# l13039968960/stm32H7-YOLO

Measured on AMD Instinct MI355X. Metric: images/sec int8 YOLO-face 56x56, higher is better.
Workload: dtype int8; 1 GPU; BASELINE configs[1]: batch=4096 int8 YOLO-face 56x56x3 frames per GPU, fused LDS-resident forward + GPU box decode; frames_per_gpu=4096, global_batch=4096, frame_bytes_in=9408, frame_bytes_out=882, input_batches_rotated=8, input_bytes_resident=308281344, kernel=yoloface56_fused<F=2,NW=8>, requant_rounding=ref, parallelism=single GPU, gather_every=1, collectives_issued=0, launch_streams=2

## Files before the change

stm32h7-yolo_amd/csrc/yf_fused56.hip.h:

```cpp


template <class B, int C, int F, int NT>
__device__ __forceinline__ void dump_buf(const char* frames, int8_t* dump, long stride, long off, long first_frame,
                                         long n_frames, int tid, int ch0 = 0, int split = 1 << 30, int gap = 0) {
  if (!dump) return;
  for (int i = tid; i < F * B::P * C; i += NT) {
    const int ch = i % C; const int t = i / C;
    const int p = t % B::P; const int f = t / B::P;
    if (first_frame + f >= n_frames) continue;
    const int phys = ch0 + ch + (ch >= split ? gap : 0);
    dump[(first_frame + f) * stride + off + (long)p * C + ch] = (int8_t)frames[f * B::FS + B::at_p(p) + phys];
  }
}

template <class B, int C, int FT, int NT, class IdOf>
__device__ __forceinline__ void dump_sets(const char* frames, int8_t* dump, long stride, long off, const IdOf& id_of, int tid, int ch0 = 0, int split = 1 << 30, int gap = 0) {
  for (int i = tid; i < FT * B::P * C; i += NT) {
    const int ch = i % C; const int t = i / C;
    const int p = t % B::P; const int f = t / B::P;
    const long id = id_of(f);
    if (id < 0) continue;
    const int phys = ch0 + ch + (ch >= split ? gap : 0);
    dump[id * stride + off + (long)p * C + ch] = (int8_t)frames[f * B::FS + B::at_p(p) + phys];
  }
}

struct DumpOffsets {
  enum { T1 = 0, T2 = T1 + 6272, T3 = T2 + 6272, T4 = T3 + 3136, Q21 = T4 + 14112, T6 = Q21 + 3528, T7 = T6 + 3528,
         T8 = T7 + 1176, T9 = T8 + 7056, T11 = T9 + 7056, T14 = T11 + 1176, T15 = T14 + 7056, Q45 = T15 + 4704,
         T17 = Q45 + 1176, T18 = T17 + 1176, T19 = T18 + 392, T20 = T19 + 1960, T22 = T20 + 1960, T23 = T22 + 392,
         T24 = T23 + 1960, T26 = T24 + 1960, T30 = T26 + 392, T31 = T30 + 2352, T32 = T31 + 1960, T33 = T32 + 1960,
         P8 = T33 + 1568, C17 = P8 + 3528, P25 = C17 + 1176, C34 = P25 + 1176, C40 = C34 + 392, L43 = C40 + 392,
         TOTAL = L43 + 1176 };
};

struct NetParams {
  const int8_t* in;
  int8_t* out;
  long n;
  const uint8_t* tab;
  int8_t* dump;
  int stop_stage;
  yf_det* dets;
  int* counts;
  int cap, mode;
  int q_thr;
  float w_scale, h_scale;
  char* scratch;
};
static_assert(sizeof(yf_table_index) <= YF_INDEX_RESERVED, "index does not fit its reserved slot");
typedef const __attribute__((address_space(4))) char* kargs_ptr;
__device__ __forceinline__ kargs_ptr kargs_here() {
  kargs_ptr p = (kargs_ptr)__builtin_amdgcn_kernarg_segment_ptr();
  asm volatile("" : "+s"(p));
  return p;
}
#define YF_ARG(FIELD) (*reinterpret_cast<const __attribute__((address_space(4))) decltype(NetParams::FIELD)*>(kargs_here() + offsetof(NetParams, FIELD)))

#ifndef YF_POOL_MERGE
#define YF_POOL_MERGE 1
#endif
#ifndef YF_POOL8H_WAVES
#define YF_POOL8H_WAVES 3
#endif
#ifndef YF_POOL8V_WAVES
#define YF_POOL8V_WAVES 3
#endif
#ifndef YF_PRIO_LIST
#define YF_PRIO_LIST 3,3,3,3,3,3,3,3,3,3, 2,2,2,2, 1,1,1,1,1,1, 0,0,0,0,0,0,0
#endif
constexpr int STAGE_PRIO[27] = {YF_PRIO_LIST};
template <int K> __device__ __forceinline__ void stage_prio() {
  if constexpr (K == 0 || STAGE_PRIO[K] != STAGE_PRIO[K - 1]) __builtin_amdgcn_s_setprio(STAGE_PRIO[K]);
}
#if defined(YF_LAB) && defined(YF_DUMP_PROD_ORDER)
#define YF_PDUMP 1
#else
#define YF_PDUMP 0
#endif
template <bool DUMP> constexpr bool tail_batch() { return !DUMP || YF_PDUMP; }

template <int F, int NW, bool DUMP, bool CAM = false>
#if !defined(YF_LAB) || !defined(YF_TPJ13)
#undef YF_TPJ13
#define YF_TPJ13 3
#endif
#if !defined(YF_LAB) || !defined(YF_TPJ23)
#undef YF_TPJ23
#define YF_TPJ23 2
#endif
#if defined(YF_LAB) && defined(YF_WHATIF_WPE)
#define YF_WPE(NW) YF_WHATIF_WPE
#else
#define YF_WPE(NW) ((NW) == 12 ? 6 : (NW) >= 8 ? 4 : ((NW) == 6 ? 3 : 2))
#endif
__global__ void __launch_bounds__(NW * 64, YF_WPE(NW)) yoloface56_fused(const NetParams prm) {
  extern __shared__ __attribute__((aligned(16))) char smem[];
  constexpr int NT = NW * 64;
  constexpr bool BATCH = tail_batch<DUMP>();
  constexpr bool POOL_MERGE = YF_POOL_MERGE != 0 && (!DUMP || YF_PDUMP) && NW >= 8;
  constexpr bool XDUMP = DUMP && !YF_PDUMP;
  typedef Buf<B_T14::OFF, 14, 14, 32, 14, 0, 0> B_T6X;
  typedef typename std::conditional<POOL_MERGE, B_T6X, B_T6>::type B_T6M;
  constexpr int FT = BATCH ? 2 * F : F;
  typedef TailBufs<BATCH ? FRAME_STRIDE / 2 : FRAME_STRIDE> U;
  constexpr int OUT_ALL_BYTES = BATCH ? 0 : (F * OUT_FRAME_BYTES + 15) & ~15;
  static_assert(std::is_same<decltype(&yoloface56_fused<F, NW, DUMP, CAM>), void (*)(const NetParams)>::value, "YF_ARG: NetParams is the kernel's only argument (kernarg offset 0)");
  uint8_t* luts = reinterpret_cast<uint8_t*>(smem);
  constexpr int PRE = v2::pre_bytes<F, tail_batch<DUMP>()>();
  char* out_all = smem + PRE;
  char* frames = smem + PRE + OUT_ALL_BYTES;
  const int n_frames = (int)prm.n;
  const int tid0 = threadIdx.x;
  const uint8_t* __restrict__ tab = prm.tab;
  int vz = 0;
  asm volatile("" : "+v"(vz));
  const __attribute__((address_space(1))) uint8_t* lut_src = (const __attribute__((address_space(1))) uint8_t*)(tab + PLAN.lut_off);
  asm volatile("" : "+s"(lut_src));
  for (int i = tid0; i < v2::LUT_B / 16; i += NT)
    reinterpret_cast<v4u*>(luts)[i] = *(const __attribute__((address_space(1))) v4u*)(lut_src + (uint32_t)(16 * i));
  for (int i = tid0; i < v2::ZERO_B / 16; i += NT) reinterpret_cast<uint4*>(smem + v2::ZERO)[i] = uint4{0, 0, 0, 0};
  constexpr int DBG_LUT = PRE + OUT_ALL_BYTES + FRAME_BYTES + (F - 1) * FRAME_STRIDE;
  if constexpr (DUMP) { if (tid0 < YF_DBG_LUT_BYTES / 16) reinterpret_cast<v4u*>(smem + DBG_LUT)[tid0] = *(const __attribute__((address_space(1))) v4u*)(lut_src + (uint32_t)(YF_N_LUT * 256 + YF_ADDLUT_BYTES + 16 * tid0)); }
#if !(defined(YF_LAB) && defined(YF_WHATIF_NO_PROLOGUE_TABLES))
  {
    typedef v2::JobTabs<F, tail_batch<DUMP>()> JTS;
    typedef typename JTS::U UT;
    v2::fill_jobtab<F, 1, B_T1, B_T2, JTS::JT_DW3>(smem, tid0);
    v2::fill_jobtab<F, 2, B_T4, B_T6M, JTS::JT_DW10>(smem, tid0);
    v2::fill_jobtab<F, 1, B_T8, B_T9, JTS::JT_DW15>(smem, tid0);
    v2::fill_jobtab<JTS::FT, 2, typename UT::T15, typename UT::T17, JTS::JT_DW27>(smem, tid0);
    v2::fill_jobtab<JTS::FT, 1, typename UT::T19, typename UT::T20, JTS::JT_DW32>(smem, tid0);
    typedef v2::HaloTabs<F, tail_batch<DUMP>()> HTS;
    v2::build_halotab<typename HTS::G1, HTS::H_T1, NT>(smem, tid0);
    v2::build_halotab<typename HTS::G4, HTS::H_T4, NT>(smem, tid0);
    v2::build_halotab<typename HTS::G8, HTS::H_T8, NT>(smem, tid0);
    v2::build_halotab<typename HTS::G15, HTS::H_T15, NT>(smem, tid0);
    v2::build_halotab<typename HTS::G19, HTS::H_T19, NT>(smem, tid0);
  }
#endif

  auto sfresh = [](int v) { asm volatile("" : "+s"(v)); return v; };
  auto n_groups = [&]() { return (int)((uint32_t)(sfresh(n_frames) + F - 1) / (uint32_t)F); };
  int gstep = (int)gridDim.x;
  asm volatile("" : "+s"(gstep));
  auto park_slot = [&]() { return YF_ARG(scratch) + (uint32_t)(sfresh((int)blockIdx.x) * (F * TailBufs<FRAME_BYTES>::T15_BYTES)); };
  const AddK no_add = {};
  auto addctx = [&](int k) {
    const uint8_t* a = tab + offsetof(yf_table_index, add) + k * sizeof(yf_add);
    return AddK{uniform_u32(a + offsetof(yf_add, mo2)), uniform_u32(a + offsetof(yf_add, zro)),
                (unsigned long)uniform_u32(a + offsetof(yf_add, c64o)) | ((unsigned long)uniform_u32(a + offsetof(yf_add, c64o) + 4) << 32),
                (int)uniform_u32(a + offsetof(yf_add, rso))};
  };
  constexpr long DS = DumpOffsets::TOTAL;
#ifdef YF_BARPROF
  bool prof_on = false;
  int bar_no = 0;
  long long* prof_out = reinterpret_cast<long long*>(prm.dump) + ((long)blockIdx.x * NW + __builtin_amdgcn_readfirstlane(tid0 >> 6)) * 80;
#define YF_SYNC() do { asm volatile("s_waitcnt vmcnt(0)" ::: "memory");    \
                       if (prof_on && (tid0 & 63) == 0 && bar_no < 40) prof_out[2 * bar_no] = __builtin_readcyclecounter(); __syncthreads(); \
                       if (prof_on && (tid0 & 63) == 0 && bar_no < 40) prof_out[2 * bar_no + 1] = __builtin_readcyclecounter(); ++bar_no; } while (0)
#else
#define YF_SYNC() do { asm volatile("s_waitcnt vmcnt(0)" ::: "memory"); __syncthreads(); } while (0)
#endif
#define YF_HALO(B, RING, FR, G, HOFF, WI, TID) \
  do { int ht_ = TID; asm volatile("" : "+v"(ht_)); \
       v2::fill_halo_t<B, typename v2::HaloTabs<F, BATCH>::G, v2::HaloTabs<F, BATCH>::HOFF>(frames, load_halo_zp(tab, WI), ht_); } while (0)
#define YF_FETCH(CS, WV, LN) v2::fetch_consts_s<CS>(tab, WV, LN)
#define YF_CONV1(WV, LN, CS) v2::conv1_2_stage<F, NW, CS>(frames, tab, WV, LN)
#define YF_DENSE(FR, TPJ, KS, BW, IN, OUT, CH0, COUT, EPI, LUT, ADDB, DI, AD, WV, LN, CS) \
  v2::dense2_stage<FR, NW, TPJ, KS, BW, IN, OUT, CH0, COUT, EPI, LUT, ADDB, CS>(frames, out_all, tab, AD, WV, LN)
#define YF_DW(FR, STRIDE, IN, OUT, C, LUT, WI, WV, LN, CS, JTOFF) v2::dw2_stage<FR, NW, STRIDE, IN, OUT, C, LUT, CS, v2::JobTabs<F, BATCH>::JTOFF>(frames, tab, WV, LN)
#define YF_DUMP(BUF, C, OFF, ...) \
  if constexpr (DUMP) { if (prm.dump) { dump_buf<BUF, C, F, NT>(frames, prm.dump, DS, DumpOffsets::OFF, first, n_frames, tid, ##__VA_ARGS__); YF_SYNC(); } }
  int stage_no = 0;
#define YF_STAGE_END() if constexpr (DUMP) { if (++stage_no == prm.stop_stage) continue; }
#define YF_PRIO(K) stage_prio<K>()

  int prev_first = -1;
  auto decode_prev = [&](int w, int ln) {
    if (prm.dets != nullptr && prev_first >= 0 && w >= NW - F && prev_first + (w - (NW - F)) < n_frames) {
      int dl = ln;
      asm volatile("" : "+v"(dl));
      yfdec::decode_frame(reinterpret_cast<const int8_t*>(out_all) + (w - (NW - F)) * OUT_FRAME_BYTES, prev_first + (w - (NW - F)), dl,
                          prm.mode, prm.w_scale, prm.h_scale, prm.dets, prm.counts, prm.cap);
    }
  };
  constexpr int PARKED = (int)0x80000000;
  for (int st = blockIdx.x; (st & ~PARKED) < n_groups(); st += gstep) {
    const int grp = st & ~PARKED;
    const int first = grp * F;
#ifdef YF_BARPROF
    bar_no = 0;
    prof_on = !DUMP && prm.dump != nullptr && grp == (int)blockIdx.x + gstep;
#endif
    int tid = tid0, tid_f = tid0, tid_m = tid0, tid_t = tid0;
    if constexpr ((YF_LAUNDER & 1) != 0) asm volatile("" : "+v"(tid_f));
    if constexpr ((YF_LAUNDER & 2) != 0) asm volatile("" : "+v"(tid_m));
    if constexpr ((YF_LAUNDER & 4) != 0) asm volatile("" : "+v"(tid_t));
    const int lane = tid & 63;
    const int wave = __builtin_amdgcn_readfirstlane(tid >> 6);
    const int L_f = tid_f & 63, L_m = tid_m & 63, L_t = tid_t & 63;
    const int W_f = __builtin_amdgcn_readfirstlane(tid_f >> 6), W_m = __builtin_amdgcn_readfirstlane(tid_m >> 6), W_t = __builtin_amdgcn_readfirstlane(tid_t >> 6);
    (void)lane; (void)wave;
#if !defined(YF_BARPROF)
    asm volatile("s_waitcnt lgkmcnt(0)\n\ts_barrier" ::: "memory");
#else
    YF_SYNC();
#endif
    stage_no = 0;
    YF_PRIO(0);
    int tid_s = tid0;
    asm volatile("" : "+v"(tid_s));
    if constexpr (CAM) stage_input_cam<F, NT>(frames, reinterpret_cast<const uint8_t*>(YF_ARG(in)), first, n_frames, (int)uniform_u32(tab + offsetof(yf_table_index, in_zp)), tid_s);
    else stage_input<F, NT>(frames, YF_ARG(in), first, n_frames, (int)uniform_u32(tab + offsetof(yf_table_index, in_zp)), tid_s);
    YF_FETCH(0, W_f, L_f);
    YF_HALO(B_T1, true, F, G1, H_T1, YF_W_DW3, tid_f);
    YF_SYNC();
    YF_STAGE_END()
    YF_PRIO(1);
    YF_FETCH(1, W_f, L_f);
    YF_CONV1(W_f, L_f, 0);
    YF_SYNC(); YF_DUMP(B_T1, 8, T1)
    YF_STAGE_END()
    YF_PRIO(2);
    YF_FETCH(2, W_f, L_f);
    YF_DW(F, 1, B_T1, B_T2, 8, YF_L_LEAKY4, YF_W_DW3, W_f, L_f, 1, JT_DW3);
    YF_SYNC(); YF_DUMP(B_T2, 8, T2)
    YF_STAGE_END()
    YF_PRIO(3);
    YF_FETCH(3, W_f, L_f);
    YF_DENSE(F, 1, 1, 8, B_T2, B_T3, 0, 4, EPI_RAW, 0, B_T3, YF_D_C5, no_add, W_f, L_f, 2);
    YF_SYNC(); YF_DUMP(B_T3, 4, T3)
    YF_STAGE_END()
    YF_PRIO(4);
    YF_HALO(B_T4, false, F, G4, H_T4, YF_W_DW10, tid_f);
    YF_FETCH(4, W_f, L_f);
    YF_DENSE(F, 5, 1, 4, B_T3, B_T4, 0, 18, EPI_LUT, YF_L_LEAKY7, B_T4, YF_D_C6, no_add, W_f, L_f, 3);
    YF_SYNC(); YF_DUMP(B_T4, 18, T4)
    YF_STAGE_END()
    if constexpr (POOL_MERGE) {
      constexpr int PH = YF_POOL8H_WAVES, PV = YF_POOL8V_WAVES;
      YF_PRIO(5);
      YF_FETCH(5, W_m, L_m);
      if (W_m < PH) {
        if constexpr (F == 2) pool8_h_rows<F, PH>(frames, W_m, L_m);
        else pool8_h<F, PH * 64>(frames, tid_m);
      } else v2::dw2_stage<F, NW - PH, 2, B_T4, B_T6M, 18, YF_L_LEAKY11, 4, v2::JobTabs<F, BATCH>::JT_DW10>(frames, tab, W_m - PH, L_m);
      YF_SYNC(); YF_DUMP(B_T6M, 18, T6)
      YF_PRIO(8);
      YF_FETCH(6, W_m, L_m);
      YF_DENSE(F, 1, 2, 16, B_T6M, B_T7, 0, 6, EPI_RAW, 0, B_T7, YF_D_C12, no_add, W_m, L_m, 5);
      YF_SYNC(); YF_DUMP(B_T7, 6, T7)
      YF_PRIO(9);
      YF_HALO(B_T8, true, F, G8, H_T8, YF_W_DW15, tid_m);
      YF_FETCH(7, W_m, L_m);
      if (W_m < PV) pool8_v<F, PV * 64, false>(frames, tid_m);
      else v2::dense2_stage<F, NW - PV, YF_TPJ13, 1, 8, B_T7, B_T8, 0, 36, EPI_LUT, YF_L_LEAKY14, B_T8, 6>(frames, out_all, tab, no_add, W_m - PV, L_m);
      YF_SYNC(); YF_DUMP(B_T14, 18, Q21) YF_DUMP(B_T8, 36, T8)
    } else {
  YF_PRIO(5);
#if !(defined(YF_LAB) && defined(YF_WHATIF_NO_POOL8H))
      pool8_h<F, NT>(frames, tid_f);
      YF_SYNC();
#endif
      YF_STAGE_END()
      YF_PRIO(6);
      pool8_v<F, NT, XDUMP>(frames, tid_m);
      YF_SYNC();
      YF_PRIO(7);
      YF_FETCH(5, W_m, L_m);
      YF_DW(F, 2, B_T4, B_T6, 18, YF_L_LEAKY11, YF_W_DW10, W_m, L_m, 4, JT_DW10);
      YF_SYNC(); YF_DUMP(B_T14, 18, Q21) YF_DUMP(B_T14, 18, P8, YF_T14_CONV_BASE) YF_DUMP(B_T6, 18, T6)
      YF_STAGE_END()
      YF_PRIO(8);
      YF_FETCH(6, W_m, L_m);
      YF_DENSE(F, 1, 2, 16, B_T6, B_T7, 0, 6, EPI_RAW, 0, B_T7, YF_D_C12, no_add, W_m, L_m, 5);
      YF_SYNC(); YF_DUMP(B_T7, 6, T7)
      YF_STAGE_END()
      YF_PRIO(9);
      YF_HALO(B_T8, true, F, G8, H_T8, YF_W_DW15, tid_m);
      YF_FETCH(7, W_m, L_m);
      YF_DENSE(F, YF_TPJ13, 1, 8, B_T7, B_T8, 0, 36, EPI_LUT, YF_L_LEAKY14, B_T8, YF_D_C13, no_add, W_m, L_m, 6);
      YF_SYNC(); YF_DUMP(B_T8, 36, T8)
      YF_STAGE_END()
    }
    YF_PRIO(10);
    YF_FETCH(8, W_m, L_m);
    YF_DW(F, 1, B_T8, B_T9, 36, YF_L_LEAKY16, YF_W_DW15, W_m, L_m, 7, JT_DW15);
    YF_SYNC(); YF_DUMP(B_T9, 36, T9)
    YF_STAGE_END()
    YF_PRIO(11);
    YF_FETCH(9, W_m, L_m);
    if constexpr (XDUMP)
      v2::dense2_stage<F, NW, 1, 3, 16, B_T9, B_T11, 0, 6, EPI_ADD, YF_A_ADD18, B_T7, 8, B_T14::OFF + YF_T14_CONV_BASE, B_T14::S>(frames, out_all, tab, addctx(YF_A_ADD18), W_m, L_m);
    else
    YF_DENSE(F, 1, 3, 16, B_T9, B_T11, 0, 6, EPI_ADD, YF_A_ADD18, B_T7, YF_D_C17, addctx(YF_A_ADD18), W_m, L_m, 8);
    YF_SYNC(); YF_DUMP(B_T11, 6, T11) if constexpr (XDUMP) { YF_DUMP(B_T14, 6, C17, YF_T14_CONV_BASE) }
    YF_STAGE_END()
    YF_PRIO(12);
    YF_FETCH(10, W_m, L_m);
    YF_DENSE(F, 3, 1, 8, B_T11, B_T14, YF_T14_CONV_BASE, 18, EPI_LUT, YF_L_LEAKY20, B_T14, YF_D_C19, no_add, W_m, L_m, 9);
    YF_SYNC(); YF_DUMP(B_T14, 36, T14, 0, 18, 2)
    YF_STAGE_END()
    YF_PRIO(13);
    if constexpr (BATCH) {
#if !(defined(YF_LAB) && defined(YF_WHATIF_FS))
      static_assert(U::T15::FS >= U::T15_BYTES && B_T9::OFF <= U::T15::FS && U::T15::FS + U::T15_BYTES <= B_T14::OFF,
                    "the odd sets' T15 lands on T9 / T11 (dead), clear of conv2d_23's input (concat_22) and output (the even sets' T15)");
#endif
      if (st < 0) {
        constexpr int PV = TailBufs<FRAME_BYTES>::T15_BYTES / 16, WI = (PV + 63) / 64;
        const char* park = park_slot();
        for (int j = W_m; j < F * WI; j += NW) {
          const int f = j / WI, k0 = (j - f * WI) * 64;
          if (k0 + L_m < PV)
            __builtin_amdgcn_global_load_lds((const __attribute__((address_space(1))) void*)(uintptr_t)(park + (uint32_t)((f * PV + k0 + L_m) * 16)),
                                             (__attribute__((address_space(3))) void*)(uintptr_t)(uint32_t)(PRE + (2 * f + 1) * U::T15::FS + 16 * k0),
                                             16, 0, 0);
        }
      }
    }
    YF_HALO(B_T15, false, F, G15, H_T15, YF_W_DW27, tid_m);
    YF_FETCH(11, W_m, L_m);
    YF_DENSE(F, YF_TPJ23, 3, 16, B_T14, B_T15, 0, 24, EPI_LUT, YF_L_LEAKY24, B_T15, YF_D_C23, no_add, W_m, L_m, 10);
    if constexpr (BATCH) asm volatile("s_waitcnt vmcnt(0)" ::: "memory");
    YF_SYNC(); YF_DUMP(B_T15, 24, T15)
    YF_STAGE_END()
    int odd_first = -1;
    if constexpr (BATCH) {
      constexpr int V = U::T15_BYTES / 16;
      static_assert(U::T15_BYTES == TailBufs<FRAME_BYTES>::T15_BYTES, "one slot size for the park stores and the DMA back");
      if (st >= 0 && grp + gstep < n_groups()) {
        char* park = park_slot();
        __builtin_assume(tid_t >= 0 && tid_t < NT);
        for (int i = tid_t; i < F * V; i += NT) {
          const int f = i / V, k = i - f * V;
          *reinterpret_cast<uint4*>(park + (uint32_t)(16 * i)) = *reinterpret_cast<const uint4*>(frames + f * FRAME_STRIDE + 16 * k);
        }
        st |= PARKED;
        continue;
      }
      if (st < 0) {
        odd_first = (grp - gstep) * F;
        st &= ~PARKED;
      }
    }
    const int first_t = sfresh(grp) * F;
    auto frame_of = [&](int f) -> int {
      int id = first_t + f;
      if constexpr (BATCH) id = (f & 1) ? (odd_first >= 0 ? odd_first + (f >> 1) : -1) : first_t + (f >> 1);
      return id < n_frames ? id : -1;
    };
#define YF_DUMP_T(BUF, C, OFF, ...) \
  if constexpr (DUMP) { if (prm.dump) { if constexpr (BATCH) dump_sets<BUF, C, FT, NT>(frames, prm.dump, DS, DumpOffsets::OFF, frame_of, tid, ##__VA_ARGS__); \
                                        else dump_buf<BUF, C, FT, NT>(frames, prm.dump, DS, DumpOffsets::OFF, first, n_frames, tid, ##__VA_ARGS__); \
                                        YF_SYNC(); } }
    YF_PRIO(14);
    YF_FETCH(12, W_t, L_t);
    {
      constexpr int PW = v2::pool25_waves<FT>();
      static_assert(PW < NW, "waves left for conv2d_27");
      if (W_t < PW) v2::pool25_cols<FT, typename U::T15, typename U::T30, XDUMP>(frames, W_t * 64 + L_t);
      else v2::dw2_stage<FT, NW - PW, 2, typename U::T15, typename U::T17, 24, YF_L_LEAKY28, 11, v2::JobTabs<F, BATCH>::JT_DW27>(frames, tab, W_t - PW, L_t);
    }
    YF_SYNC(); YF_DUMP_T(typename U::T30, 24, Q45) if constexpr (XDUMP) { YF_DUMP_T(typename U::T30, 24, P25, 24) } YF_DUMP_T(typename U::T17, 24, T17)
    YF_STAGE_END()
    YF_PRIO(15);
    YF_FETCH(13, W_t, L_t);
    YF_DENSE(FT, 1, 2, 16, typename U::T17, typename U::T18, 0, 8, EPI_RAW, 0, typename U::T18, YF_D_C29, no_add, W_t, L_t, 12);
    if constexpr (!BATCH) decode_prev(W_t, L_t);
    YF_SYNC(); YF_DUMP_T(typename U::T18, 8, T18)
    YF_STAGE_END()
    YF_PRIO(16);
    YF_HALO(typename U::T19, true, FT, G19, H_T19, YF_W_DW32, tid_t);
    YF_FETCH(14, W_t, L_t);
    YF_DENSE(FT, 5, 1, 8, typename U::T18, typename U::T19, 0, 40, EPI_LUT, YF_L_LEAKY31, typename U::T19, YF_D_C30, no_add, W_t, L_t, 13);
    YF_SYNC(); YF_DUMP_T(typename U::T19, 40, T19)
    YF_STAGE_END()
    YF_PRIO(17);
    YF_FETCH(15, W_t, L_t);
    YF_DW(FT, 1, typename U::T19, typename U::T20, 40, YF_L_LEAKY33, YF_W_DW32, W_t, L_t, 14, JT_DW32);
    YF_SYNC(); YF_DUMP_T(typename U::T20, 40, T20)
    YF_STAGE_END()
    YF_PRIO(18);
    YF_FETCH(16, W_t, L_t);
    if constexpr (XDUMP)
      v2::dense2_stage<FT, NW, 1, 3, 16, typename U::T20, typename U::T22, 0, 8, EPI_ADD, YF_A_ADD35, typename U::T18, 15, U::T30::OFF + 24, U::T30::S>(frames, out_all, tab, addctx(YF_A_ADD35), W_t, L_t);
    else
    YF_DENSE(FT, 1, 3, 16, typename U::T20, typename U::T22, 0, 8, EPI_ADD, YF_A_ADD35, typename U::T18, YF_D_C34, addctx(YF_A_ADD35), W_t, L_t, 15);
    YF_SYNC(); YF_DUMP_T(typename U::T22, 8, T22) if constexpr (XDUMP) { YF_DUMP_T(typename U::T30, 8, C34, 24) }
    YF_STAGE_END()
    YF_PRIO(19);
    YF_HALO(typename U::T19, true, FT, G19, H_T19, YF_W_DW38, tid_t);
    YF_FETCH(17, W_t, L_t);
    YF_DENSE(FT, 5, 1, 8, typename U::T22, typename U::T19, 0, 40, EPI_LUT, YF_L_LEAKY37, typename U::T19, YF_D_C36, no_add, W_t, L_t, 16);
    YF_SYNC(); YF_DUMP_T(typename U::T19, 40, T23)
    YF_STAGE_END()
    YF_PRIO(20);
    YF_FETCH(18, W_t, L_t);
    YF_DW(FT, 1, typename U::T19, typename U::T20, 40, YF_L_LEAKY39, YF_W_DW38, W_t, L_t, 17, JT_DW32);
    YF_SYNC(); YF_DUMP_T(typename U::T20, 40, T24)
    YF_STAGE_END()
    YF_PRIO(21);
    YF_FETCH(19, W_t, L_t);
    if constexpr (XDUMP)
      v2::dense2_stage<FT, NW, 1, 3, 16, typename U::T20, typename U::T26, 0, 8, EPI_ADD, YF_A_ADD41, typename U::T22, 18, U::T30::OFF + 24, U::T30::S>(frames, out_all, tab, addctx(YF_A_ADD41), W_t, L_t);
    else
    YF_DENSE(FT, 1, 3, 16, typename U::T20, typename U::T26, 0, 8, EPI_ADD, YF_A_ADD41, typename U::T22, YF_D_C40, addctx(YF_A_ADD41), W_t, L_t, 18);
    YF_SYNC(); YF_DUMP_T(typename U::T26, 8, T26) if constexpr (XDUMP) { YF_DUMP_T(typename U::T30, 8, C40, 24) }
    YF_STAGE_END()
    YF_PRIO(22);
    YF_FETCH(20, W_t, L_t);
    if constexpr (XDUMP)
      v2::dense2_stage<FT, NW, 2, 1, 8, typename U::T26, typename U::T30, 24, 24, EPI_LUT, YF_L_L43Q44, typename U::T30, 19, U::T20::OFF, U::T20::S, DBG_LUT>(frames, out_all, tab, no_add, W_t, L_t);
    else
    YF_DENSE(FT, 3, 1, 8, typename U::T26, typename U::T30, 24, 24, EPI_LUT, YF_L_L43Q44, typename U::T30, YF_D_C42, no_add, W_t, L_t, 19);
    YF_SYNC(); YF_DUMP_T(typename U::T30, 48, T30) if constexpr (XDUMP) { YF_DUMP_T(typename U::T20, 24, L43) }
    YF_STAGE_END()
    YF_PRIO(23);
    YF_HALO(typename U::T19, true, FT, G19, H_T19, YF_W_DW49, tid_t);
    YF_FETCH(21, W_t, L_t);
    YF_DENSE(FT, 2, 3, 16, typename U::T30, typename U::T19, 0, 40, EPI_LUT, YF_L_LEAKY48, typename U::T19, YF_D_C47, no_add, W_t, L_t, 20);
    YF_SYNC(); YF_DUMP_T(typename U::T19, 40, T31)
    YF_STAGE_END()
    YF_PRIO(24);
    YF_FETCH(22, W_t, L_t);
    YF_DW(FT, 1, typename U::T19, typename U::T20, 40, YF_L_LEAKY50, YF_W_DW49, W_t, L_t, 21, JT_DW32);
    YF_SYNC(); YF_DUMP_T(typename U::T20, 40, T32)
    YF_STAGE_END()
    YF_PRIO(25);
    YF_FETCH(23, W_t, L_t);
    if (BATCH && YF_ARG(dets) != nullptr && W_t < 2) {
      int dl = L_t;
      asm volatile("" : "+v"(dl));
      const uint8_t* src = reinterpret_cast<const uint8_t*>(sfresh(W_t) == 0 ? yfdec::d_sig_bits : yfdec::d_exp_bits);
      const uint32_t voff = 16u * (uint32_t)dl;
      const uint32_t dst = (uint32_t)(PRE + OUT_ALL_BYTES + 1024 * W_t);
      uint32_t keep;
      asm volatile("s_mov_b32 %0, m0\n\ts_mov_b32 m0, %3\n\ts_nop 0\n\tglobal_load_lds_dwordx4 %1, %2\n\ts_mov_b32 m0, %0"
                   : "=&s"(keep) : "v"(voff), "s"(src), "s"(dst) : "memory");
    }
    YF_DENSE(FT, 2, 3, 16, typename U::T20, typename U::T33, 0, 32, EPI_LUT, YF_L_LEAKY52, typename U::T33, YF_D_C51, no_add, W_t, L_t, 22);
    YF_SYNC(); YF_DUMP_T(typename U::T33, 32, T33)
    YF_STAGE_END()
    YF_PRIO(26);
    if constexpr (!BATCH) {
      YF_DENSE(FT, 1, 2, 16, typename U::T33, typename U::T33, 0, 18, EPI_HEAD, 0, typename U::T33, YF_D_C53, no_add, W_t, L_t, 23);
      YF_SYNC();
      const int n16 = min(F, n_frames - first) * (OUT_FRAME_BYTES / 2);
      int8_t* dst = YF_ARG(out) + (size_t)(uint32_t)first * OUT_FRAME_BYTES;
      const uint16_t* srcp = reinterpret_cast<const uint16_t*>(out_all);
      for (int i = tid; i < n16; i += NT) *reinterpret_cast<uint16_t*>(dst + (uint32_t)(2 * i)) = srcp[i];
      prev_first = first;
    } else {
      YF_DENSE(FT, 1, 2, 16, typename U::T33, typename U::HEAD, 0, 18, EPI_HEAD_LDS, 0, typename U::T33, YF_D_C53, no_add, W_t, L_t, 23);
      YF_SYNC();
      constexpr int H16 = OUT_FRAME_BYTES / 2;
      yf_det* const dets = YF_ARG(dets);
      int8_t* const heads = YF_ARG(out);
      const bool split = dets != nullptr && FT < NW;
      const int c0 = split ? tid_t - FT * 64 : tid_t, cstep = split ? NT - FT * 64 : NT;
      if (!split || W_t >= FT) {
#pragma unroll
        for (int f = 0; f < FT; ++f) {
          const int id = frame_of(f);
          if (id >= 0) {
            int8_t* dst = heads + (size_t)(uint32_t)id * OUT_FRAME_BYTES;
            for (int k = c0; k < H16; k += cstep)
              *reinterpret_cast<uint16_t*>(dst + (uint32_t)(2 * k)) = *reinterpret_cast<const uint16_t*>(frames + f * U::HEAD::FS + U::HEAD::OFF + 2 * k);
          }
        }
// ... 38 lines not shown
```

stm32h7-yolo_amd/csrc/yf_kernels.hip.h:

```cpp
#include <hip/hip_runtime.h>
#include <stddef.h>
#include <stdint.h>
#include <type_traits>
#include "yf_tables.h"

#pragma clang diagnostic push
#pragma clang diagnostic ignored "-Wint-to-pointer-cast"
#if !defined(YF_LAB) || !defined(YF_LAUNDER)
#undef YF_LAUNDER
#define YF_LAUNDER 0
#endif
#define YF_ROW_SKEW 4
#define YF_T8_ROW_SKEW 32
namespace YF_NS {

#ifndef YF_NOINLINE_STAGES
#define YF_STAGE_FN __device__ __forceinline__
#else
#define YF_STAGE_FN __device__ __attribute__((noinline))
#endif

typedef int v4i __attribute__((ext_vector_type(4)));
typedef short v2s __attribute__((ext_vector_type(2)));

// ... 211 lines not shown
  return v;
}
constexpr int ACC0 = YF_ACC_OFFSET;
#ifdef YF_RQ3_DENSE
constexpr bool DENSE_SIGNLESS = true;
#else
constexpr bool DENSE_SIGNLESS = false;
#endif
#ifdef YF_RQ_FP32
constexpr bool RQ_FP32 = true;
#else
constexpr bool RQ_FP32 = false;
#endif
__device__ __forceinline__ v4i acc_init(const v4u zr) {
  if constexpr (RQ_FP32) return (v4i)zr;
  else { (void)zr; return v4i{ACC0, ACC0, ACC0, ACC0}; }
}
__device__ __forceinline__ int any_value() { int u; asm volatile("" : "=v"(u)); return u; }
__device__ __forceinline__ int clampi(int v, int lo, int hi) { return min(max(v, lo), hi); }
__device__ __forceinline__ uint32_t join4(uint32_t b0, uint32_t b1, uint32_t b2, uint32_t b3) {
  uint32_t lo, hi, v;
  asm("v_lshl_or_b32 %0, %1, 8, %2" : "=v"(lo) : "v"(b1), "v"(b0));
  asm("v_lshl_or_b32 %0, %1, 8, %2" : "=v"(hi) : "v"(b3), "v"(b2));
  asm("v_lshl_or_b32 %0, %1, 16, %2" : "=v"(v) : "v"(hi), "v"(lo));
  return v;
}
typedef const __attribute__((address_space(3))) uint8_t* lds_u8_ptr;
template <int LUT_ID>
__device__ __forceinline__ uint32_t lutb(int idx) {
  return *(lds_u8_ptr)(uint32_t)(LUT_ID * 256 + idx);
}
__device__ __forceinline__ uint32_t pkmax(uint32_t a, uint32_t b) {
  v2s x, y; __builtin_memcpy(&x, &a, 4); __builtin_memcpy(&y, &b, 4);
  v2s r = __builtin_elementwise_max(x, y);
  uint32_t o; __builtin_memcpy(&o, &r, 4); return o;
}
__device__ __forceinline__ uint32_t pk_shl8(uint32_t d) {
  v2s x; __builtin_memcpy(&x, &d, 4);
  x = x << 8;
  uint32_t o; __builtin_memcpy(&o, &x, 4); return o;
}
struct SplitB {
  uint32_t o, e;
  __device__ __forceinline__ SplitB() : o(0x80008000u), e(0x80008000u) {}
  __device__ __forceinline__ explicit SplitB(uint32_t d) : o(d), e(pk_shl8(d)) {}
  __device__ __forceinline__ SplitB mx(const SplitB& b) const { SplitB r; r.o = pkmax(o, b.o); r.e = pkmax(e, b.e); return r; }
  __device__ __forceinline__ uint32_t merge() const { return __builtin_amdgcn_perm(o, e, 0x07030501u); }
  __device__ __forceinline__ uint32_t b3() const { return o >> 24; }
  __device__ __forceinline__ uint32_t b2() const { return e >> 24; }
  __device__ __forceinline__ uint32_t b1() const { return (o >> 8) & 255u; }
  __device__ __forceinline__ uint32_t b0() const { return (e >> 8) & 255u; }
};
template <int LUT_ID>
__device__ __forceinline__ uint32_t lut4_raw(const SplitB& v) {
  return join4(lutb<LUT_ID>(v.b0()), lutb<LUT_ID>(v.b1()), lutb<LUT_ID>(v.b2()), lutb<LUT_ID>(v.b3()));
}

__device__ __forceinline__ uint32_t lds_u32(const char* p) { return *reinterpret_cast<const uint32_t*>(p); }
typedef const __attribute__((address_space(4))) v4i* cv4i_ptr;
typedef const __attribute__((address_space(4))) uint32_t* cu32_ptr;
typedef const __attribute__((address_space(4))) v4ul* cv4ul_ptr;
struct I4 { int x, y, z, w; };
__device__ __forceinline__ I4 uniform_int4(const void* p) { const v4i v = *(cv4i_ptr)(uintptr_t)p; return I4{v[0], v[1], v[2], v[3]}; }
__device__ __forceinline__ uint32_t uniform_u32(const void* p) { return *(cu32_ptr)(uintptr_t)p; }
struct PassV { v4u m2, zr; };
#ifdef YF_LAB
__device__ __forceinline__ PassV load_pass_v(const uint8_t* pass, int vz) {
  const v4u* p = reinterpret_cast<const v4u*>(pass + vz);
  return PassV{p[0], p[1]};
}
__device__ __forceinline__ v4i load_wfrag(const uint8_t* p, int vz) {
  (void)vz;
  return *reinterpret_cast<const v4i*>(p);
}
#endif
struct PassS { v4ul c64; v4i rs; };
#ifdef YF_LAB
__device__ __forceinline__ PassS load_pass_s(const uint8_t* pass) {
  return PassS{*(cv4ul_ptr)(uintptr_t)(pass + 32), *(cv4i_ptr)(uintptr_t)(pass + 64)};
}
#endif
struct TablePlan { int w_off[YF_N_DENSE], c_off[YF_N_DENSE], g_off[YF_N_DW], lut_off, total;
                   int vb_off[YF_N_CS], vb_bytes[YF_N_CS], sb_off[YF_N_CS]; };
constexpr int PLAN_COUT[YF_N_DENSE] = {8, 4, 18, 6, 36, 6, 18, 24, 8, 40, 8, 40, 8, 24, 40, 32, 18};
constexpr int PLAN_KROW[YF_N_DENSE] = {YF_CONV1_KROW, 16, 16, 32, 16, 48, 16, 48, 32, 16, 48, 16, 48, 16, 48, 48, 32};
constexpr int PLAN_DWC[YF_N_DW] = {8, 18, 36, 24, 40, 40, 40};
constexpr int plan_passes(int cs) { return yf_cs_dense[cs] >= 0 ? (PLAN_COUT[yf_cs_dense[cs]] + 3) / 4 : (PLAN_DWC[yf_cs_dw[cs]] + 3) / 4; }
constexpr int plan_wbytes(int cs) { return yf_cs_dense[cs] >= 0 ? ((PLAN_COUT[yf_cs_dense[cs]] + 3) & ~3) * PLAN_KROW[yf_cs_dense[cs]] : 0; }
constexpr TablePlan make_plan() {
  TablePlan p = {};
  int off = YF_INDEX_RESERVED;
  for (int i = 0; i < YF_N_DENSE; ++i) {
    const int cp = (PLAN_COUT[i] + 3) & ~3;
    off = (off + 15) & ~15; p.w_off[i] = off; off += cp * PLAN_KROW[i];
    off = (off + 15) & ~15; p.c_off[i] = off; off += (cp / 4) * (int)sizeof(yf_pass);
  }
  for (int i = 0; i < YF_N_DW; ++i) { off = (off + 15) & ~15; p.g_off[i] = off; off += ((PLAN_DWC[i] + 3) / 4) * YF_DW_GROUP_BYTES; }
  off = (off + 15) & ~15; p.lut_off = off; off += YF_N_LUT * 256 + YF_ADDLUT_BYTES + YF_DBG_LUT_BYTES;
  for (int cs = 0; cs < YF_N_CS; ++cs) {
    const int bytes = yf_cs_dense[cs] >= 0 ? plan_wbytes(cs) + plan_passes(cs) * (int)sizeof(yf_pass_v) + (yf_cs_add[cs] >= 0 ? 2048 : 0)
                                           : plan_passes(cs) * YF_DWV_GROUP_BYTES;
    off = (off + 15) & ~15; p.vb_off[cs] = off; p.vb_bytes[cs] = (bytes + 15) & ~15; off += p.vb_bytes[cs];
  }
  for (int cs = 0; cs < YF_N_CS; ++cs) { off = (off + 15) & ~15; p.sb_off[cs] = off; off += plan_passes(cs) * (int)sizeof(yf_pass_s); }
  off = (off + 15) & ~15; off += 64;
  p.total = off;
  return p;
}
constexpr TablePlan PLAN = make_plan();
#ifdef YF_LAB
__device__ __forceinline__ yf_dense load_dense(const uint8_t*, int i) {
  yf_dense d = {};
  d.w_off = (uint32_t)PLAN.w_off[i]; d.c_off = (uint32_t)PLAN.c_off[i];
  return d;
}
__device__ __forceinline__ yf_dw load_dw(const uint8_t*, int i) {
  yf_dw d = {};
  d.g_off = (uint32_t)PLAN.g_off[i];
  return d;
}
#endif
__device__ __forceinline__ int load_halo_zp(const uint8_t* tab, int i) {
  return (int)uniform_u32(tab + offsetof(yf_table_index, halo_zp) + 4 * i);
}

template <int JOBS, int NW>
__device__ __forceinline__ void job_range(int wave, int& j0, int& j1) {
  constexpr int BASE = JOBS / NW, REM = JOBS % NW;
  j0 = wave * BASE + min(wave, REM);
  j1 = j0 + BASE + (wave < REM ? 1 : 0);
}

template <class B, bool RING, int F, int NT>
YF_STAGE_FN void fill_halo(char* frames, int zp, int tid) {
  const uint32_t v = (uint32_t)(zp & 255) * 0x01010101u;
  constexpr int DW = B::S / 4;
  constexpr int HR = B::H + B::PT + (RING ? 1 : 0), WR = B::RS;
  constexpr int NPIX = RING ? (2 * WR + 2 * (HR - 2)) : (WR + HR - 1);
  for (int i = tid; i < F * NPIX * DW; i += NT) {
    const int d = i % DW, t = i / DW, k = t % NPIX, f = t / NPIX;
    int r, c;
    if constexpr (RING) {
      if (k < WR) { r = 0; c = k; }
      else if (k < 2 * WR) { r = HR - 1; c = k - WR; }
      else { const int m = k - 2 * WR; r = 1 + (m >> 1); c = (m & 1) ? WR - 1 : 0; }
    } else {
      if (k < WR) { r = 0; c = k; } else { r = 1 + (k - WR); c = 0; }
    }
    *reinterpret_cast<uint32_t*>(frames + f * B::FS + B::OFF + r * B::ROWB + c * B::S + 4 * d) = v;
  }
}

__device__ __forceinline__ uint32_t funnel(uint32_t hi, uint32_t lo, int sh) { return __builtin_amdgcn_alignbit(hi, lo, sh); }
template <int F, int NT>
YF_STAGE_FN void stage_input(char* frames, const int8_t* __restrict__ in, int first_frame, int n_frames,
                                            int zp, int tid) {
  const uint32_t hv = (uint32_t)(zp & 255) * 0x01010101u;
  constexpr int RSW = B_IN::RS, HH = B_IN::H, WQ = B_IN::W / 4;
  constexpr int PER_FRAME = HH * WQ, TOTAL = F * PER_FRAME, ITERS = (TOTAL + NT - 1) / NT;
  for (int i = tid; i < F * (RSW + HH); i += NT) {
    const int f = i / (RSW + HH), k = i - f * (RSW + HH);
    const int idx = k < RSW ? k : (k - RSW + 1) * RSW + 3;
    *reinterpret_cast<uint32_t*>(frames + f * B_IN::FS + B_IN::OFF + idx * 4) = hv;
  }
  const int lastf = min(n_frames - 1 - first_frame, F - 1);
  const int8_t* base = in + (size_t)(uint32_t)first_frame * IN_FRAME_BYTES;
  static_assert(RSW == B_IN::W + 4 && B_IN::S == 4, "dst = OFF + 16 * (r + y + RSW/4 + 1) relies on rows of W + 4 dwords");
  uint32_t ld[ITERS][3];
#pragma unroll
  for (int it = 0; it < ITERS; ++it) {
    const int i = min(tid + it * NT, TOTAL - 1);
    int f = 0;
#pragma unroll
    for (int k = 1; k < F; ++k) f += (i >= k * PER_FRAME) ? 1 : 0;
    const int r = i - f * PER_FRAME;
    const uint32_t* src = reinterpret_cast<const uint32_t*>(base + (uint32_t)(min(f, lastf) * PER_FRAME + r) * 12u);
    ld[it][0] = src[0]; ld[it][1] = src[1]; ld[it][2] = src[2];
  }
#pragma unroll
  for (int it = 0; it < ITERS; ++it) {
    const int i = tid + it * NT;
    if (ITERS * NT == TOTAL || i < TOTAL) {
      int f = 0;
#pragma unroll
      for (int k = 1; k < F; ++k) f += (i >= k * PER_FRAME) ? 1 : 0;
      const int r = i - f * PER_FRAME;
      uint4 px;
      px.x = ld[it][0];
      px.y = funnel(ld[it][1], ld[it][0], 24);
      px.z = funnel(ld[it][2], ld[it][1], 16);
      px.w = ld[it][2] >> 8;
      const int y = (int)((uint32_t)r / (uint32_t)WQ);
      *reinterpret_cast<uint4*>(frames + f * B_IN::FS + B_IN::OFF + (RSW + 4) * 4 + 16 * (r + y)) = px;
    }
  }
}

constexpr int CAM_FRAME_BYTES = 112 * 112 * 2;
__device__ __forceinline__ uint32_t cam_pixel(uint32_t s0, uint32_t s1) {
  const uint32_t r = ((s0 >> 11) & 0x001F001Fu) + ((s1 >> 11) & 0x001F001Fu);
  const uint32_t g = ((s0 >> 5) & 0x003F003Fu) + ((s1 >> 5) & 0x003F003Fu);
  const uint32_t b = (s0 & 0x001F001Fu) + (s1 & 0x001F001Fu);
  const uint32_t rs = r + (r >> 16), gs = g + (g >> 16), bs = b + (b >> 16);
  return (((rs & 0x7Cu) << 1) | ((gs & 0xFCu) << 8) | ((bs & 0x7Cu) << 17)) ^ 0x00808080u;
}
template <int F, int NT>
YF_STAGE_FN void stage_input_cam(char* frames, const uint8_t* __restrict__ cam, int first_frame, int n_frames, int zp, int tid) {
  const uint32_t hv = (uint32_t)(zp & 255) * 0x01010101u;
  constexpr int RSW = B_IN::RS, HH = B_IN::H, WQ = B_IN::W / 4;
  constexpr int PER_FRAME = HH * WQ, TOTAL = F * PER_FRAME;
  for (int i = tid; i < F * (RSW + HH); i += NT) {
    const int f = i / (RSW + HH), k = i - f * (RSW + HH);
    const int idx = k < RSW ? k : (k - RSW + 1) * RSW + 3;
    *reinterpret_cast<uint32_t*>(frames + f * B_IN::FS + B_IN::OFF + idx * 4) = hv;
  }
  const int lastf = min(n_frames - 1 - first_frame, F - 1);
  const uint8_t* base = cam + (size_t)(uint32_t)first_frame * CAM_FRAME_BYTES;
  constexpr int ITERS = (TOTAL + NT - 1) / NT;
  auto item = [&](int i, int& f, int& r, int& y, const uint8_t*& src) {
    f = 0;
#pragma unroll
    for (int k = 1; k < F; ++k) f += (i >= k * PER_FRAME) ? 1 : 0;
    r = i - f * PER_FRAME;
    y = (int)((uint32_t)r / (uint32_t)WQ);
    const int xq = r - y * WQ;
    src = base + (uint32_t)(min(f, lastf) * CAM_FRAME_BYTES + (2 * y) * 224 + 16 * xq);
  };
  auto commit = [&](int f, int r, int y, const uint4& a, const uint4& c) {
    constexpr uint32_t SWAP = 0x02030001u;
    uint4 px;
    px.x = cam_pixel(__builtin_amdgcn_perm(a.x, a.x, SWAP), __builtin_amdgcn_perm(c.x, c.x, SWAP));
    px.y = cam_pixel(__builtin_amdgcn_perm(a.y, a.y, SWAP), __builtin_amdgcn_perm(c.y, c.y, SWAP));
    px.z = cam_pixel(__builtin_amdgcn_perm(a.z, a.z, SWAP), __builtin_amdgcn_perm(c.z, c.z, SWAP));
    px.w = cam_pixel(__builtin_amdgcn_perm(a.w, a.w, SWAP), __builtin_amdgcn_perm(c.w, c.w, SWAP));
    *reinterpret_cast<uint4*>(frames + f * B_IN::FS + B_IN::OFF + (RSW + 4) * 4 + 16 * (r + y)) = px;
  };
#pragma unroll
  for (int it = 0; it < ITERS; it += 2) {
    const int i0 = tid + it * NT, i1 = i0 + NT;
    int f0, r0, y0, f1, r1, y1;
    const uint8_t *s0, *s1;
    item(min(i0, TOTAL - 1), f0, r0, y0, s0);
    item(min(i1, TOTAL - 1), f1, r1, y1, s1);
    const uint4 a0 = *reinterpret_cast<const uint4*>(s0), c0 = *reinterpret_cast<const uint4*>(s0 + 224);
    const uint4 a1 = *reinterpret_cast<const uint4*>(s1), c1 = *reinterpret_cast<const uint4*>(s1 + 224);
    if (i0 < TOTAL) commit(f0, r0, y0, a0, c0);
    if (it + 1 < ITERS && i1 < TOTAL) commit(f1, r1, y1, a1, c1);
  }
}

struct AddK { uint32_t mo2, zro; unsigned long c64o; int rso; };

#ifdef YF_LAB
#include "yf_lab_stages.hip.h"
#endif

template <int NO, int LIM, class LOADC, class STORE>
__device__ __forceinline__ void pool8_sweep(int o0, LOADC loadc, STORE store) {
  constexpr int NR = NO + 3;
  SplitB r[NR];
#pragma unroll
  for (int jj = 0; jj < NR; ++jj) {
    const int j = o0 - 2 + jj;
    r[jj] = SplitB(loadc(clampi(2 * j + 1, 0, LIM))).mx(SplitB(loadc(clampi(2 * j + 2, 0, LIM))));
  }
  SplitB q[NR - 1];
#pragma unroll
  for (int jj = 0; jj < NR - 1; ++jj) q[jj] = r[jj].mx(r[jj + 1]);
#pragma unroll
  for (int n = 0; n < NO; ++n) store(o0 + n, q[n].mx(q[n + 2]));
}
template <int F, int NT>
YF_STAGE_FN void pool8_h(char* frames, int tid) {
  constexpr int NO = 5, OW = B_HB::W, IH = B_T4::H, NCH = (OW + NO - 1) / NO;
  __builtin_assume(tid >= 0 && tid < NT);
  for (int i = tid; i < F * IH * NCH * 5; i += NT) {
    const int cg = i % 5; int t = i / 5;
    const int k = t % NCH; t /= NCH;
    const int y = t % IH; const int f = t / IH;
    char* fbase = frames + f * B_T4::FS;
    const char* row = fbase + B_T4::at(y, 0) + 4 * cg;
    char* dst = fbase + B_HB::OFF + (y * OW) * 20 + 4 * cg;
    pool8_sweep<NO, B_T4::W - 1>(min(k * NO, OW - NO),
                                 [&](int x) { return lds_u32(row + x * B_T4::S); },
                                 [&](int ox, const SplitB& v) { *reinterpret_cast<uint32_t*>(dst + ox * 20) = v.merge(); });
  }
}
#if YF_H0 == 56
template <int F>
constexpr bool pool8_rows_conflict_free(int arena0) {
  constexpr int NO = 5, OW = B_HB::W, IH = B_T4::H;
  if (F != 2 || IH > 32) return false;
  for (int f = 0; f < F; ++f)
    for (int k = 0; k < (OW + NO - 1) / NO; ++k)
      for (int cg = 0; cg < 5; ++cg)
        for (int jj = 0; jj < 2 * (NO + 3); ++jj) {
          const int o0 = k * NO < OW - NO ? k * NO : OW - NO, x0 = 2 * (o0 - 2 + jj / 2) + 1 + jj % 2, x = x0 < 0 ? 0 : x0 > B_T4::W - 1 ? B_T4::W - 1 : x0;
          int addr[32] = {};
          for (int l = 0; l < 32; ++l) {
            const int y = l < IH ? l : IH - 1;
            addr[l] = arena0 + f * B_T4::FS + B_T4::OFF + (y + B_T4::PT) * B_T4::ROWB + (x + B_T4::PL) * B_T4::S + 4 * cg;
          }
          if (!lds_conflict_free<4>(addr)) return false;
        }
  return true;
}
template <int F, int PH>
YF_STAGE_FN void pool8_h_rows(char* frames, int wave, int lane) {
  constexpr int NO = 5, OW = B_HB::W, IH = B_T4::H;
  static_assert(F == 2 && PH == 3 && PH * NO >= OW && IH <= 32, "one wave per chunk of five outputs, one frame per half-wave");
  asm volatile("" : "+v"(lane));
  const int y = lane & 31;
  if (y < IH) {
    char* fbase = frames + (lane >> 5) * B_T4::FS;
    const char* row = fbase + B_T4::at(y, 0);
    char* dst = fbase + B_HB::OFF + y * (OW * 20);
    auto pass = [&](auto o0) {
#pragma nounroll
      for (int cg = 0; cg < 5; ++cg)
        pool8_sweep<NO, B_T4::W - 1>(decltype(o0)::value,
                                     [&](int x) { return lds_u32(row + 4 * cg + x * B_T4::S); },
                                     [&](int ox, const SplitB& v) { *reinterpret_cast<uint32_t*>(dst + 4 * cg + ox * 20) = v.merge(); });
    };
    if (wave == 0) pass(std::integral_constant<int, 0>());
    else if (wave == 1) pass(std::integral_constant<int, NO>());
    else pass(std::integral_constant<int, OW - NO>());
  }
}
#endif
template <int F, int NT, bool STASH = false>
YF_STAGE_FN void pool8_v(char* frames, int tid) {
  constexpr int NO = 5, OW = B_HB::W, OH = B_T14::H, NCH = (OH + NO - 1) / NO;
  static_assert(OH >= NO, "column shorter than one sweep");
  __builtin_assume(tid >= 0 && tid < NT);
  for (int i = tid; i < F * OW * NCH * 5; i += NT) {
    const int cg = i % 5; int t = i / 5;
    const int k = t % NCH; t /= NCH;
    const int ox = t % OW; const int f = t / OW;
    char* fbase = frames + f * B_HB::FS;
    const char* col = fbase + B_HB::OFF + ox * 20 + 4 * cg;
    char* dst = fbase + B_T14::OFF + ox * B_T14::S + 4 * cg;
    pool8_sweep<NO, B_HB::H - 1>(min(k * NO, OH - NO),
                                 [&](int r) { return lds_u32(col + r * (OW * 20)); },
                                 [&](int oy, const SplitB& v) {
                                   *reinterpret_cast<uint32_t*>(dst + oy * (OW * B_T14::S)) = lut4_raw<YF_L_Q21>(v);
                                   if constexpr (STASH) *reinterpret_cast<uint32_t*>(dst + oy * (OW * B_T14::S) + YF_T14_CONV_BASE) = v.merge();
                                 });
  }
}

namespace v2 {
constexpr int LUT_B = YF_N_LUT * 256;
constexpr int JT = LUT_B, JT_B = 896;
constexpr int ZERO = JT + JT_B, ZERO_B = 640;
constexpr int SLOT0 = ZERO + ZERO_B, SLOT_B = 2816;
constexpr int slot(int cs) { return SLOT0 + (cs & 1) * SLOT_B; }
struct Lay56 {
  static constexpr int ZERO = v2::ZERO, JT = v2::JT, JT_BYTES = v2::JT_B;
  static constexpr int slot(int cs) { return v2::slot(cs); }
};
constexpr int max_block() { int m = 0; for (int i = 0; i < YF_N_CS; ++i) m = PLAN.vb_bytes[i] > m ? PLAN.vb_bytes[i] : m; return m; }
static_assert(max_block() <= SLOT_B && SLOT0 % 16 == 0 && SLOT_B % 16 == 0, "a constant block fits a ring slot");

typedef const __attribute__((address_space(3))) v4i* lds_v4i_ptr;
typedef const __attribute__((address_space(3))) v4u* lds_v4u_ptr;
typedef const __attribute__((address_space(3))) uint32_t* lds_u32_ptr;
typedef const __attribute__((address_space(3))) v2u* lds_u2_ptr;
__device__ __forceinline__ v4i lds_v4i(uint32_t a) { return *(lds_v4i_ptr)a; }
__device__ __forceinline__ v4u lds_v4u(uint32_t a) { return *(lds_v4u_ptr)a; }

template <int CS, class LAY = Lay56, int BYTES_ = -1>
__device__ __forceinline__ void fetch_consts(const uint8_t* __restrict__ tab, int wave, int lane) {
  constexpr int BYTES = BYTES_ >= 0 ? BYTES_ : PLAN.vb_bytes[CS], NCHUNK = (BYTES + 1023) / 1024;
  if (wave < NCHUNK) {
    asm volatile("" : "+v"(lane));
    const int off = wave * 1024 + lane * 16;
    if (off < BYTES) {
      const uint8_t* src = tab + PLAN.vb_off[CS] + off;
      const uint32_t dst = (uint32_t)(LAY::slot(CS) + wave * 1024);
      uint32_t keep;
      asm volatile("s_mov_b32 %0, m0\n\ts_mov_b32 m0, %2\n\ts_nop 0\n\tglobal_load_lds_dwordx4 %1, off\n\ts_mov_b32 m0, %0"
                   : "=&s"(keep) : "v"(src), "s"(dst) : "memory");
    }
  }
}
template <int CS>
__device__ __forceinline__ void fetch_consts_s(const uint8_t* __restrict__ tab, int wave, int lane) {
  constexpr int BYTES = PLAN.vb_bytes[CS], NCHUNK = (BYTES + 1023) / 1024;
  asm volatile("" : "+s"(wave));
  if (wave < NCHUNK) {
    asm volatile("" : "+v"(lane));
    const int off = wave * 1024 + lane * 16;
    if (off < BYTES) {
      const uint32_t voff = (uint32_t)(PLAN.vb_off[CS] + off);
      const uint32_t dst = (uint32_t)(Lay56::slot(CS) + wave * 1024);
      uint32_t keep;
      asm volatile("s_mov_b32 %0, m0\n\ts_mov_b32 m0, %3\n\ts_nop 0\n\tglobal_load_lds_dwordx4 %1, %2\n\ts_mov_b32 m0, %0"
                   : "=&s"(keep) : "v"(voff), "s"(tab), "s"(dst) : "memory");
// ... 537 lines not shown
```

Baseline: 33.08 million images/s.

## Overlap halo fill with input loads and tighten barrier waitcnt

Moves the T1 halo fill into the input staging routine so it runs while the global input loads are still in flight, instead of after them. Replaces the inline-asm vmcnt wait in the stage barrier with a builtin s_waitcnt encoding, which lets the compiler see and schedule the wait. Rewrites the T15 park reload as hand-written global_load_lds inline asm with explicit M0 save and restore, to avoid compiler-generated M0 setup overhead. The asm path relies on the M0 handling and the waitcnt encoding being correct for this target.

```diff
diff --git a/stm32h7-yolo_amd/csrc/yf_fused56.hip.h b/stm32h7-yolo_amd/csrc/yf_fused56.hip.h
--- a/stm32h7-yolo_amd/csrc/yf_fused56.hip.h
+++ b/stm32h7-yolo_amd/csrc/yf_fused56.hip.h
@@ -157,11 +157,11 @@
   bool prof_on = false;
   int bar_no = 0;
   long long* prof_out = reinterpret_cast<long long*>(prm.dump) + ((long)blockIdx.x * NW + __builtin_amdgcn_readfirstlane(tid0 >> 6)) * 80;
-#define YF_SYNC() do { asm volatile("s_waitcnt vmcnt(0)" ::: "memory");    \
+#define YF_SYNC() do { asm volatile("" ::: "memory"); __builtin_amdgcn_s_waitcnt(0x0F70);    \
                        if (prof_on && (tid0 & 63) == 0 && bar_no < 40) prof_out[2 * bar_no] = __builtin_readcyclecounter(); __syncthreads(); \
                        if (prof_on && (tid0 & 63) == 0 && bar_no < 40) prof_out[2 * bar_no + 1] = __builtin_readcyclecounter(); ++bar_no; } while (0)
 #else
-#define YF_SYNC() do { asm volatile("s_waitcnt vmcnt(0)" ::: "memory"); __syncthreads(); } while (0)
+#define YF_SYNC() do { asm volatile("" ::: "memory"); __builtin_amdgcn_s_waitcnt(0x0F70); __syncthreads(); } while (0)
 #endif
 #define YF_HALO(B, RING, FR, G, HOFF, WI, TID) \
   do { int ht_ = TID; asm volatile("" : "+v"(ht_)); \
@@ -212,10 +212,10 @@
     YF_PRIO(0);
     int tid_s = tid0;
     asm volatile("" : "+v"(tid_s));
-    if constexpr (CAM) stage_input_cam<F, NT>(frames, reinterpret_cast<const uint8_t*>(YF_ARG(in)), first, n_frames, (int)uniform_u32(tab + offsetof(yf_table_index, in_zp)), tid_s);
-    else stage_input<F, NT>(frames, YF_ARG(in), first, n_frames, (int)uniform_u32(tab + offsetof(yf_table_index, in_zp)), tid_s);
+    auto halo_t1 = [&]() { YF_HALO(B_T1, true, F, G1, H_T1, YF_W_DW3, tid_f); };
+    if constexpr (CAM) stage_input_cam<F, NT>(frames, reinterpret_cast<const uint8_t*>(YF_ARG(in)), first, n_frames, (int)uniform_u32(tab + offsetof(yf_table_index, in_zp)), tid_s, halo_t1);
+    else stage_input<F, NT>(frames, YF_ARG(in), first, n_frames, (int)uniform_u32(tab + offsetof(yf_table_index, in_zp)), tid_s, halo_t1);
     YF_FETCH(0, W_f, L_f);
-    YF_HALO(B_T1, true, F, G1, H_T1, YF_W_DW3, tid_f);
     YF_SYNC();
     YF_STAGE_END()
     YF_PRIO(1);
@@ -314,10 +314,13 @@
         const char* park = park_slot();
         for (int j = W_m; j < F * WI; j += NW) {
           const int f = j / WI, k0 = (j - f * WI) * 64;
-          if (k0 + L_m < PV)
-            __builtin_amdgcn_global_load_lds((const __attribute__((address_space(1))) void*)(uintptr_t)(park + (uint32_t)((f * PV + k0 + L_m) * 16)),
-                                             (__attribute__((address_space(3))) void*)(uintptr_t)(uint32_t)(PRE + (2 * f + 1) * U::T15::FS + 16 * k0),
-                                             16, 0, 0);
+          if (k0 + L_m < PV) {
+            const uint32_t voff = (uint32_t)((f * PV + k0 + L_m) * 16);
+            const uint32_t dst = (uint32_t)(PRE + (2 * f + 1) * U::T15::FS + 16 * k0);
+            uint32_t keep;
+            asm volatile("s_mov_b32 %0, m0\n\ts_mov_b32 m0, %3\n\ts_nop 0\n\tglobal_load_lds_dwordx4 %1, %2\n\ts_mov_b32 m0, %0"
+                         : "=&s"(keep) : "v"(voff), "s"(park), "s"(dst) : "memory");
+          }
         }
       }
     }
diff --git a/stm32h7-yolo_amd/csrc/yf_kernels.hip.h b/stm32h7-yolo_amd/csrc/yf_kernels.hip.h
--- a/stm32h7-yolo_amd/csrc/yf_kernels.hip.h
+++ b/stm32h7-yolo_amd/csrc/yf_kernels.hip.h
@@ -387,9 +387,10 @@
 }
 
 __device__ __forceinline__ uint32_t funnel(uint32_t hi, uint32_t lo, int sh) { return __builtin_amdgcn_alignbit(hi, lo, sh); }
-template <int F, int NT>
+struct NoWork { __device__ __forceinline__ void operator()() const {} };
+template <int F, int NT, class WORK = NoWork>
 YF_STAGE_FN void stage_input(char* frames, const int8_t* __restrict__ in, int first_frame, int n_frames,
-                                            int zp, int tid) {
+                                            int zp, int tid, WORK while_in_flight = WORK()) {
   const uint32_t hv = (uint32_t)(zp & 255) * 0x01010101u;
   constexpr int RSW = B_IN::RS, HH = B_IN::H, WQ = B_IN::W / 4;
   constexpr int PER_FRAME = HH * WQ, TOTAL = F * PER_FRAME, ITERS = (TOTAL + NT - 1) / NT;
@@ -412,6 +413,7 @@
     const uint32_t* src = reinterpret_cast<const uint32_t*>(base + (uint32_t)(min(f, lastf) * PER_FRAME + r) * 12u);
     ld[it][0] = src[0]; ld[it][1] = src[1]; ld[it][2] = src[2];
   }
+  while_in_flight();
 #pragma unroll
   for (int it = 0; it < ITERS; ++it) {
     const int i = tid + it * NT;
@@ -439,8 +441,8 @@
   const uint32_t rs = r + (r >> 16), gs = g + (g >> 16), bs = b + (b >> 16);
   return (((rs & 0x7Cu) << 1) | ((gs & 0xFCu) << 8) | ((bs & 0x7Cu) << 17)) ^ 0x00808080u;
 }
-template <int F, int NT>
-YF_STAGE_FN void stage_input_cam(char* frames, const uint8_t* __restrict__ cam, int first_frame, int n_frames, int zp, int tid) {
+template <int F, int NT, class WORK = NoWork>
+YF_STAGE_FN void stage_input_cam(char* frames, const uint8_t* __restrict__ cam, int first_frame, int n_frames, int zp, int tid, WORK while_in_flight = WORK()) {
   const uint32_t hv = (uint32_t)(zp & 255) * 0x01010101u;
   constexpr int RSW = B_IN::RS, HH = B_IN::H, WQ = B_IN::W / 4;
   constexpr int PER_FRAME = HH * WQ, TOTAL = F * PER_FRAME;
@@ -479,6 +481,7 @@
     item(min(i1, TOTAL - 1), f1, r1, y1, s1);
     const uint4 a0 = *reinterpret_cast<const uint4*>(s0), c0 = *reinterpret_cast<const uint4*>(s0 + 224);
     const uint4 a1 = *reinterpret_cast<const uint4*>(s1), c1 = *reinterpret_cast<const uint4*>(s1 + 224);
+    if (it == 0) while_in_flight();
     if (i0 < TOTAL) commit(f0, r0, y0, a0, c0);
     if (it + 1 < ITERS && i1 < TOTAL) commit(f1, r1, y1, a1, c1);
   }
```

Result: no change. 33.07 million images/s, median of 5 (-0.0%).
